# TUM-PIK-ESM/Terrarium.jl

Measured on AMD Instinct MI355X. Metric: column-steps/sec, higher is better.
Workload: dtype f64

## Files before the change

### terrarium.jl_amd/csrc/terrarium_hip.hip

```cpp
#include "trm_host.hpp"

#include <dlfcn.h>

using namespace trm;
using namespace trmh;

namespace {
thread_local std::string g_create_error;
}

namespace trmh {
int fail(trm_ctx* ctx, int code, const std::string& msg) {
    if (ctx) ctx->err = msg;
    else g_create_error = msg;
    return code;
}
}

namespace {

template <class NF> struct HostGrid {
    std::vector<NF> zF, zC, dzc, rdzc, rdzf, dzf, psiz;
    NF dzf_bot, dzf_top;
    void build(int Nz, const double* thickness) {
// ... 443 lines not shown
            for (const auto& a : c->averages) {
                if (a.field != f) continue;
                if (b.count == ACC_BATCH) return fail(c, TRM_EUNSUPPORTED, "more than 32 accumulators of fields that share a field");
                AccumEntry& e = b.e[b.count++];
                e.src = c->d_acc_partial[sl];
                e.sum = a.d_sum;
                e.n = (long long)field_elems(c, f);
                e.pitch = is_3d(f) ? c->Nzp : 1;
                e.nz = is_3d(f) ? c->Nz : 1;
                e.src_double = 1;
            }
        }
        int rc = TRM_OK;
        by_bool(P::richards(c), [&](auto RICH) { rc = ColumnAccumLaunch<NF, RICH()>::run(c, dt, finalize, nsteps, aa); });
        if (!rc) rc = AverageLaunch<NF>::accumulate(c, b);
        if (rc) return rc;
        for (auto& a : c->averages) {
            if (a.field < 0) continue;
            for (int j = 0; j < nsteps; ++j) a.window += dt;
            a.steps += nsteps;
        }
        return TRM_OK;
    }
    template <int PROG> static int fused_prologue(trm_ctx* c, double dt, int nsteps) {
        if (PROG == PROG_MULTI && !c->series.empty()) return U::upload_series_rows(c, dt, nsteps);
        int rc = U::update_inputs(c, c->state, c->time);
        if (!rc && PROG == PROG_HEUN) rc = U::update_inputs(c, c->stage, c->time + dt);
        return rc;
    }
    template <int PROG> static int step_launch(trm_ctx* c, const StepPlan& plan, double dt, int fin, int nsteps) {
        if (plan.route == ROUTE_SURFACE_IN_LAUNCH) return std::is_same<NF, float>::value ? PackedLaunch::step_land(c, dt, fin) : FrontLaunch::run(c, plan, dt, fin, PROG == PROG_HEUN);
        if (plan.route == ROUTE_ACCUM_IN_LAUNCH) return multi_program_accum(c, dt, fin, nsteps);
        if (plan.route == ROUTE_LEVELS) return levels_launch<NF>(c, PROG, P::generic_bcs(c), dt, fin, nsteps);
        if (plan.route == ROUTE_PACKED) return PackedLaunch::step(c, dt, fin);
        if (plan.route == ROUTE_GENERIC) return PROG == PROG_HEUN ? GenericLaunch<NF>::heun(c, dt, fin) : GenericLaunch<NF>::step(c, dt, fin);
        int rc = TRM_OK;
        by_bool(P::richards(c), [&](auto RICH) { rc = ColumnLaunch<NF, RICH(), PROG>::run(c, plan, dt, fin, nsteps); });
        return rc;
    }
    static int fused_epilogue(trm_ctx* c, int rc, double dt, int fin, bool accumulate = true, bool deferred = false, bool psi_step = false) {
        if (!rc) c->closure_consistent = true;
        c->psi_consistent = !rc && psi_step;
        if (!rc) c->closure_deferred = deferred;
        if (!rc && accumulate) rc = accumulate_after(c, dt);
        c->tend_valid = fin != 0;
        c->top_valid = c->params.seb != 0 && !rc && tops_current(c);
        if (rc || !fin) return rc;
        if (P::coupled(c)) return V::surface_veg(c, c->state, true, false, 0.0);
        return c->params.seb ? U::surface(c, c->state, true) : TRM_OK;
    }
    template <int PROG> static int fused_launch(trm_ctx* c, double dt, int fin, int nsteps = 1, bool not_last = false, bool* interior = nullptr) {
        int rc = fused_prologue<PROG>(c, dt, nsteps);
        const StepPlan plan = P::plan_step(c, PROG, not_last, interior && *interior);
        const bool in_launch = plan.route == ROUTE_SURFACE_IN_LAUNCH, accum = plan.route == ROUTE_ACCUM_IN_LAUNCH;
        const bool surface_reads_fields = c->params.seb && !in_launch && !(c->top_valid && c->d_top3);
        if (!rc && c->closure_deferred && (surface_reads_fields || !plan.derives_unread)) rc = flush_closure(c);
        if (PROG != PROG_EULER && plan.check_entry && !rc) rc = fail(c, TRM_EINVAL, "trm_step: an interior launch must be followed by a ForwardEuler launch");
        if (!rc && plan.refusal) rc = fail(c, TRM_EINVAL, plan.refusal);
        if (!rc && PROG != PROG_MULTI && P::coupled(c)) rc = V::surface_veg(c, c->state, true, true, dt, c->opt_write_kf != 0);
        else if (!rc && PROG != PROG_MULTI && c->params.seb && !in_launch) rc = U::surface(c, c->state, true);
        if (!rc) rc = step_launch<PROG>(c, plan, dt, fin, nsteps);
        if (!rc && plan.psi_form == PSI_INTERIOR) c->interior_launches += 1;
        if (!rc && interior) *interior = plan.psi_form == PSI_INTERIOR;
        return fused_epilogue(c, rc, dt, fin, !accum, !plan.store_closure, plan.psi_step);
    }
    static bool interleave_now(trm_ctx* c, int steps_left) {
        if (c->opt_pipeline == 0 || steps_left < 2 || averaging(c) || !c->params.seb || !P::richards(c) || P::coupled(c) || c->part_n[1] <= 0) return false;
        if (!c->series.empty() || P::generic_bcs(c) || c->Nz > 64) return false;
        if (std::is_same<NF, float>::value && !P::packed_path(c)) return false;
        return c->opt_pipeline == 1;
    }
    static int land_steps_interleaved(trm_ctx* c, double dt, int nsteps, int finalize) {
        const bool top0 = c->top_valid, cc0 = c->closure_consistent;
        int rc = flush_closure(c);
        if (rc) return rc;
        {
            PartScope scope(c, 0);
            c->top_valid = top0;
            rc = U::surface(c, c->state, true);
        }
        for (int n = 0; n < nsteps && !rc; ++n) {
            const int fin = (finalize && n == nsteps - 1) ? 1 : 0;
            const bool tops = (n == 0) ? top0 : tops_current(c);
            c->closure_consistent = (n == 0) ? cc0 : true;
            rc = LandLaunch<NF>::run(c, 0, 1, dt, fin, tops);
            if (rc) break;
            if (n < nsteps - 1) {
                rc = LandLaunch<NF>::run(c, 1, 0, dt, 0, tops_current(c));
            } else {
                PartScope scope(c, 1);
                rc = step_launch<PROG_EULER>(c, P::plan_step(c, PROG_EULER, false, false), dt, fin, 1);
            }
            tick(c, dt, 1);
        }
        return fused_epilogue(c, rc, dt, finalize);
    }
    static int steps_per_launch_now(trm_ctx* c) {
        return !program_applies(c) ? 1 : (c->opt_steps_per_launch > 0 ? c->opt_steps_per_launch : P::auto_steps_per_launch(c));
    }
    static int step(trm_ctx* c, double dt, int nsteps, int finalize) {
        if (c->veg_mode == TRM_VEGETATION_STANDALONE) return veg_step(c, dt, nsteps, finalize, false);
        if (c->opt_kernel != TRM_KERNEL_FUSED || P::levels_per_lane(c) == 0)
            if (int rf = flush_closure(c)) return rf;
        const bool fused = c->opt_kernel == TRM_KERNEL_FUSED && P::levels_per_lane(c) > 0;
        const bool program_ok = program_applies(c);
        const bool avg = averaging(c), avg_in_launch = avg && program_ok && averages_in_launch(c);
        const int spl = (avg && !avg_in_launch) ? 1 : steps_per_launch_now(c);
        int n = 0, rc = TRM_OK;
        bool behind_interior = false;
        while (n < nsteps && !rc) {
            int m = std::min(spl, nsteps - n);
            const int fin = (finalize && n + m == nsteps) ? 1 : 0;
            if (!fused) {
                rc = U::update_inputs(c, c->state, c->time);
                c->top_valid = false;
                c->tend_valid = true;
                if (!rc) rc = unfused_step(c, dt, fin);
                if (!rc) c->closure_consistent = true;
                c->psi_consistent = false;
            } else if (m > 1 || (program_ok && single_step_program(c))) {
                rc = fused_launch<PROG_MULTI>(c, dt, fin, m, false, &behind_interior);
            } else if (interleave_now(c, nsteps - n)) {
                m = nsteps - n;
                rc = land_steps_interleaved(c, dt, m, finalize);
                n += m;
                continue;
            } else {
                rc = fused_launch<PROG_EULER>(c, dt, fin, 1, n + m < nsteps && !fin, &behind_interior);
            }
            if (rc) break;
            tick(c, dt, m);
            n += m;
        }
        if (behind_interior) {
            c->psi_consistent = false;
            const std::string err = c->err;
            if (!flush_closure(c) && !U::closure_hydrology(c, c->state, true, false)) (void)U::hydraulics(c, c->state);
            c->err = err;
            if (!rc) rc = fail(c, TRM_EINVAL, "trm_step: the call ended on an interior launch");
        }
        return rc;
    }

    static int copy_state_to_stage(trm_ctx* c, bool everything = false) {
        for (int f = 0; f < TRM_FIELD_COUNT; ++f) {
            if (!c->state.f[f] || !c->stage.f[f]) continue;
            if (f == TRM_FIELD_VWC_FORCING && c->stage_vwc_own) continue;
            const bool needed = everything || !is_3d(f) || f == TRM_FIELD_INTERNAL_ENERGY || f == TRM_FIELD_SATURATION_WATER_ICE ||
                                f == TRM_FIELD_TEND_INTERNAL_ENERGY || f == TRM_FIELD_TEND_SATURATION_WATER_ICE;
            if (needed) TRM_HIP(c, hipMemcpyAsync(c->stage.f[f], c->state.f[f], field_elems(c, f) * sizeof(NF), hipMemcpyDeviceToDevice, c->stream));
        }
        if (everything && c->state.kf_top && c->stage.kf_top)
            TRM_HIP(c, hipMemcpyAsync(c->stage.kf_top, c->state.kf_top, (size_t)c->Nh * sizeof(NF), hipMemcpyDeviceToDevice, c->stream));
        return TRM_OK;
    }
    static int heun_step_coupled_fused(trm_ctx* c, double dt, int finalize) {
        int rc = fused_prologue<PROG_HEUN>(c, dt, 1);
        if (!rc) rc = flush_closure(c);
        if (rc) return fused_epilogue(c, rc, dt, finalize);
        const VegView<NF> vs = P::veg_view(c, c->state);
        VegView<NF> vg = P::veg_view(c, c->stage);
        View<NF> sv = cached_view<NF>(c, c->stage);
        auto fed = [&](int field) {
            for (const auto& sr : c->series) if (!sr.is_bc && sr.field == field) return true;
            return false;
// ... 89 lines not shown
        c->closure_consistent = true;
        c->psi_consistent = false;
        c->last_program = TRM_PROGRAM_UNFUSED;
        int rc = heun_predict(c, dt);
        if (!rc) rc = heun_correct(c, dt, finalize);
        return rc;
    }
};

#define DISPATCH(c, expr) ((c)->precision == TRM_F64 ? Ops<double>::expr : Ops<float>::expr)

bool parse_env_int(const char* name, long lo, long hi, long multiple_of, long& out, std::string& err) {
    const char* e = std::getenv(name);
    if (!e) return false;
    char* end = nullptr;
    const long v = std::strtol(e, &end, 10);
    if (end == e || *end != 0 || v < lo || v > hi || (multiple_of > 1 && v % multiple_of != 0)) {
        err = std::string(name) + "=" + e + ": expected an integer in [" + std::to_string(lo) + ", " + std::to_string(hi) + "]" +
              (multiple_of > 1 ? " that is a multiple of " + std::to_string(multiple_of) : std::string());
        return false;
    }
    out = v;
    return true;
}
struct EnvSwitches {
    long field_skew = 16640, derive_default = -1, debug_placement = 0, handoff_tag_bias = 0, defer_closure = -1, interior_steps = -1;
    std::string error;
    EnvSwitches() {
        long v;
        if (parse_env_int("TRM_FIELD_SKEW", 0, 1 << 20, 256, v, error)) field_skew = v;
        if (error.empty() && parse_env_int("TRM_DERIVE_DEFAULT", 0, 5, 1, v, error)) derive_default = v;
        if (error.empty() && parse_env_int("TRM_DEBUG_PLACEMENT", 0, 1, 1, v, error)) debug_placement = v;
        if (error.empty() && parse_env_int("TRM_DEBUG_HANDOFF_TAG_BIAS", 0, 1, 1, v, error)) handoff_tag_bias = v;
        if (error.empty() && parse_env_int("TRM_DEFER_CLOSURE_STORES", 0, 1, 1, v, error)) defer_closure = v;
        if (error.empty() && parse_env_int("TRM_INTERIOR_STEPS", 0, 2, 1, v, error)) interior_steps = v;
        if (error.empty() && parse_env_int("TRM_STAGED_SMALL", 0, 1, 1, v, error)) {  }
        if (error.empty() && parse_env_int("TRM_SCALAR_INPUTS", 0, 1, 1, v, error)) {  }
    }
};
const EnvSwitches& env_switches() {
    static const EnvSwitches e;
    return e;
}
size_t field_skew_bytes() { return (size_t)env_switches().field_skew; }
int alloc_fields(trm_ctx* c, FieldSet& s) {
    for (int f = 0; f < TRM_FIELD_COUNT; ++f) {
        if (is_lazy_field(f) && c->veg_mode == TRM_VEGETATION_OFF) continue;
        if (s.f[f]) continue;
        size_t bytes = field_elems(c, f) * c->esize;
        const size_t skew = field_skew_bytes() * (size_t)(f % 32);
        TRM_HIP(c, hipMalloc(&s.raw[f], bytes + skew));
        s.f[f] = (char*)s.raw[f] + skew;
        if (env_switches().debug_placement) std::fprintf(stderr, "trm placement: field %d raw %p bytes %zu skew %zu\n", f, s.raw[f], bytes, skew);
        TRM_HIP(c, hipMemsetAsync(s.f[f], 0, bytes, c->stream));
    }
    if (!s.kf_top) {
        TRM_HIP(c, hipMalloc(&s.kf_top, (size_t)c->Nh * c->esize));
        TRM_HIP(c, hipMemsetAsync(s.kf_top, 0, (size_t)c->Nh * c->esize, c->stream));
    }
    TRM_HIP(c, hipStreamSynchronize(c->stream));
    return TRM_OK;
}

template <class NF> int upload_grid(trm_ctx* c, const double* thickness) {
    HostGrid<NF> g;
    g.build(c->Nz, thickness);
    auto up = [&](void** d, const std::vector<NF>& h) -> int {
// ... 1678 lines not shown
        if (int rf = flush_closure(c)) return rf;
    }
    switch (option) {
        case TRM_OPT_ASYNC: c->opt_async = value != 0; return TRM_OK;
        case TRM_OPT_STEP_KERNEL:
            if (value != TRM_KERNEL_FUSED && value != TRM_KERNEL_UNFUSED) break;
            c->opt_kernel = value;
            return TRM_OK;
        case TRM_OPT_WRITE_KF_EVERY_STEP: c->opt_write_kf = value != 0; return TRM_OK;
        case TRM_OPT_VWC_FORCING_FIELD: c->opt_vwc_field = value != 0; return TRM_OK;
        case TRM_OPT_PACKED_F32: c->opt_packed = value != 0; return TRM_OK;
        case TRM_OPT_DERIVE_CLOSURE_FIELDS:
            if (value < 0 || value > 5) break;
            c->opt_derive = value;
            return TRM_OK;
        case TRM_OPT_STEPS_PER_LAUNCH:
            if (value < 0 || value > 100000) break;
            c->opt_steps_per_launch = value;
            return TRM_OK;
        case TRM_OPT_PIPELINE_PARTS:
            if (value < 0 || value > 2) break;
            c->opt_pipeline = value;
            return TRM_OK;
        case TRM_OPT_SINGLE_STEP_PROGRAM:
            if (value < 0 || value > 2) break;
            c->opt_single_step = value;
            return TRM_OK;
        case TRM_OPT_BC_SIGNATURE: c->opt_bc_signature = value != 0; return TRM_OK;
        case TRM_OPT_ZERO_GRADIENT_FAST: c->opt_zero_gradient_fast = value != 0; c->args_valid = false; return TRM_OK;
        case TRM_OPT_SURFACE_IN_LAUNCH:
            if (value < 0 || value > 2) break;
            c->opt_front = value;
            return TRM_OK;
        case TRM_OPT_DEFER_CLOSURE_STORES: c->opt_defer_closure = value != 0; return TRM_OK;
        case TRM_OPT_INTERIOR_STEPS:
            if (value < 0 || value > 2) break;
            c->opt_interior = value;
            return TRM_OK;
        case TRM_OPT_DERIVATIVE_SERIES: c->opt_derivative_series = value != 0; return TRM_OK;
        case TRM_OPT_DERIVATIVE_SERIES_PARAMS: c->opt_derivative_series_params = value != 0; return TRM_OK;
        default: break;
    }
    return fail(c, TRM_EINVAL, "trm_set_option: unknown option or value");
}
int trm_get_option(const trm_ctx* c, int option, int* value) {
    if (!c || !value) return TRM_EINVAL;
    switch (option) {
        case TRM_OPT_ASYNC: *value = c->opt_async; return TRM_OK;
        case TRM_OPT_STEP_KERNEL: *value = c->opt_kernel; return TRM_OK;
        case TRM_OPT_WRITE_KF_EVERY_STEP: *value = c->opt_write_kf; return TRM_OK;
        case TRM_OPT_VWC_FORCING_FIELD: *value = c->opt_vwc_field; return TRM_OK;
        case TRM_OPT_PACKED_F32: *value = c->opt_packed; return TRM_OK;
        case TRM_OPT_DERIVE_CLOSURE_FIELDS: *value = c->opt_derive; return TRM_OK;
        case TRM_OPT_STEPS_PER_LAUNCH: *value = c->opt_steps_per_launch; return TRM_OK;
        case TRM_OPT_PIPELINE_PARTS: *value = c->opt_pipeline; return TRM_OK;
        case TRM_OPT_SINGLE_STEP_PROGRAM: *value = c->opt_single_step; return TRM_OK;
        case TRM_OPT_BC_SIGNATURE: *value = c->opt_bc_signature; return TRM_OK;
        case TRM_OPT_ZERO_GRADIENT_FAST: *value = c->opt_zero_gradient_fast; return TRM_OK;
        case TRM_OPT_SURFACE_IN_LAUNCH: *value = c->opt_front; return TRM_OK;
        case TRM_OPT_DEFER_CLOSURE_STORES: *value = c->opt_defer_closure; return TRM_OK;
        case TRM_INFO_CLOSURE_STORED: *value = c->closure_deferred ? 0 : 1; return TRM_OK;
        case TRM_INFO_MATERIALIZATIONS: *value = (int)c->materializations; return TRM_OK;
        case TRM_OPT_INTERIOR_STEPS: *value = c->opt_interior; return TRM_OK;
        case TRM_INFO_INTERIOR_LAUNCHES: *value = (int)c->interior_launches; return TRM_OK;
        case TRM_OPT_DERIVATIVE_SERIES: *value = c->opt_derivative_series; return TRM_OK;
        case TRM_OPT_DERIVATIVE_SERIES_PARAMS: *value = c->opt_derivative_series_params; return TRM_OK;
        case TRM_INFO_DERIVATIVE_SERIES: *value = c->derivative_series; return TRM_OK;
// ... 23 lines not shown
```

### terrarium.jl_amd/csrc/trm_host.hpp

```cpp
#pragma once
#include "../../include/terrarium_hip.h"
#include "trm_kernels.hpp"
#include "trm_column.hpp"
#include "trm_vegetation.hpp"
#include "trm_dispatch.hpp"

#include <rccl/rccl.h>

#include <cmath>
#include <limits>
#include <type_traits>
#include <cstdio>
#include <cstdlib>
#include <cstring>
#include <algorithm>
#include <string>
#include <vector>

struct FieldSet {
    void* f[TRM_FIELD_COUNT];
    void* kf_top;
    void* raw[TRM_FIELD_COUNT];
};

// ... 655 lines not shown
template <class NF, bool RICH, int H, int LPC, bool SEB, bool SERIES>
int run_column_accum(trm_ctx* c, dim3 grid, dim3 block, const View<NF>& v, const DevParams<NF>& p, const ColumnArgs<NF>& a, const AccumArgs& acc) {
    TRM_LAUNCH(c, (k_column_accum<NF, RICH, H, LPC, SEB, SERIES>), grid, block, v, p, a, acc);
    c->last_program = program_id(TRM_PROGRAM_COLUMN_MULTI, H, LPC, DERIVE_NONE, 0, 1, BCSIG_RUNTIME) | (SEB ? 1 << 25 : 0) | (SERIES ? 1 << 26 : 0) | TRM_PROGRAM_AVERAGES_IN_LAUNCH;
    return TRM_OK;
}
template <int H, int LPC, int DERIVE, bool STAGED, bool SCALAR_IN, int PROG>
int run_column_land(trm_ctx* c, dim3 grid, dim3 block, const View<double>& v, const DevParams<double>& p, const ColumnArgs<double>& a, const FrontArgs& fa) {
    TRM_LAUNCH(c, (k_column_land<double, true, H, LPC, DERIVE, STAGED, SCALAR_IN, PROG>), grid, block, v, p, a, fa);
    c->last_program = program_id(TRM_PROGRAM_COLUMN_LAND, H, LPC, DERIVE, STAGED, SCALAR_IN, BCSIG_LAND) | (PROG << 25);
    return TRM_OK;
}
template <class NF, bool RICH, int SIG> struct ColumnSigLaunch {
    static int run(trm_ctx* c, dim3 grid, dim3 block, const View<NF>& v, const DevParams<NF>& p, const ColumnArgs<NF>& a, int derive, int staged, int scalar_in);
};
template <int SIG> struct ColumnPsiLaunch {
    static int run(trm_ctx* c, dim3 grid, dim3 block, const View<double>& v, const DevParams<double>& p, const ColumnArgs<double>& a, int form, int staged, int scalar_in);
};
template <class NF, bool RICH, int SIG> struct ColumnSigHeunLaunch {
    static int run(trm_ctx* c, dim3 grid, dim3 block, const View<NF>& v, const DevParams<NF>& p, const ColumnArgs<NF>& a);
};
template <class NF> struct GenericLaunch {
    static int step(trm_ctx* c, double dt, int finalize);
    static int heun(trm_ctx* c, double dt, int finalize);
};
template <class NF, int M> struct LevelsLaunch { static int run(trm_ctx* c, int prog, bool generic, double dt, int finalize, int nsteps); };
template <class NF> inline int levels_launch(trm_ctx* c, int prog, bool generic, double dt, int finalize, int nsteps = 1) {
    return Policy<NF>::levels_per_lane(c) == 4 ? LevelsLaunch<NF, 4>::run(c, prog, generic, dt, finalize, nsteps) : LevelsLaunch<NF, 2>::run(c, prog, generic, dt, finalize, nsteps);
}
template <class NF> struct LandLaunch { static int run(trm_ctx* c, int qcol, int qsurf, double dt, int finalize, bool top_arrays); };
template <> int LandLaunch<double>::run(trm_ctx* c, int qcol, int qsurf, double dt, int finalize, bool top_arrays);
template <> int LandLaunch<float>::run(trm_ctx* c, int qcol, int qsurf, double dt, int finalize, bool top_arrays);
struct PackedLaunch {
    static int step(trm_ctx* c, double dt, int finalize);
    static int step_land(trm_ctx* c, double dt, int finalize);
};
int front_args(trm_ctx* c, const char* kernel, FrontArgs& fa);
struct FrontLaunch {
    static int run(trm_ctx* c, const StepPlan& plan, double dt, int finalize, bool heun = false);
    template <int H> static int run_hyd(trm_ctx* c, const StepPlan& plan, double dt, int finalize, bool heun);
};

#ifndef TRM_SINGLE_STEP_PROGRAM_MAX_COLUMNS
#define TRM_SINGLE_STEP_PROGRAM_MAX_COLUMNS 0
#endif

constexpr int kAccumField[ACC_SLOTS] = {
    TRM_FIELD_INTERNAL_ENERGY, TRM_FIELD_SATURATION_WATER_ICE, TRM_FIELD_TEMPERATURE, TRM_FIELD_LIQUID_WATER_FRACTION, TRM_FIELD_PRESSURE_HEAD,
    TRM_FIELD_SURFACE_EXCESS_WATER, TRM_FIELD_WATER_TABLE, TRM_FIELD_SKIN_TEMPERATURE, TRM_FIELD_GROUND_HEAT_FLUX, TRM_FIELD_SURFACE_SHORTWAVE_UP,
    TRM_FIELD_SURFACE_LONGWAVE_UP, TRM_FIELD_SURFACE_NET_RADIATION, TRM_FIELD_SENSIBLE_HEAT_FLUX, TRM_FIELD_LATENT_HEAT_FLUX,
    TRM_FIELD_EVAPORATION_GROUND, TRM_FIELD_INFILTRATION, TRM_FIELD_SURFACE_RUNOFF};
inline int accum_slot(int field) {
    for (int s = 0; s < ACC_SLOTS; ++s) if (kAccumField[s] == field) return s;
    return -1;
}
inline int accum_field(int slot) { return kAccumField[slot]; }

template <class NF> struct StepPolicy : Policy<NF> {
    using P = Policy<NF>;
    static bool tops_current(const trm_ctx* c) { return c->d_top3 != nullptr && !c->top_escaped; }
    static bool averaging(const trm_ctx* c) {
        for (const auto& a : c->averages) if (a.field >= 0) return true;
        return false;
    }
    static bool averages_in_launch(const trm_ctx* c) {
        if (c->Nz > 64 || c->part >= 0) return false;
// ... 13 lines not shown
    static bool interior_capable(const trm_ctx* c) {
        if (!std::is_same<NF, double>::value || !c->opt_interior || !c->psi_consistent || c->closure_escaped) return false;
        if (c->opt_interior == 2 && (size_t)6 * (size_t)c->Nh * (size_t)c->Nzp * sizeof(NF) > ((size_t)256 << 20)) return false;
        if (!c->opt_write_kf) return false;
        if (!P::richards(c) || c->params.seb || P::coupled(c) || c->veg_mode == TRM_VEGETATION_STANDALONE) return false;
        if (c->opt_kernel != TRM_KERNEL_FUSED || P::levels_per_lane(c) != 1 || c->part >= 0 || P::generic_bcs(c)) return false;
        if (!c->opt_bc_signature || P::hyd(c) == HYD_GENERIC || !column_psi_supported(bc_signature_of(c))) return false;
        if (averaging(c) || c->d_tan[0]) return false;
        return P::template derive_now<true>(c) == DERIVE_T_LIQ;
    }
    static bool surface_in_launch(const trm_ctx* c, bool heun = false) {
        if (c->opt_front == 0 || (heun && std::is_same<NF, float>::value)) return false;
        if (!c->params.seb || !P::richards(c) || P::coupled(c) || c->Nz > 64 || P::generic_bcs(c) || c->part >= 0) return false;
        if (c->opt_kernel != TRM_KERNEL_FUSED || !c->opt_bc_signature || bc_signature_of(c) != BCSIG_LAND) return false;
        if (P::hyd(c) != HYD_BC_LINEAR && P::hyd(c) != HYD_VG_N2) return false;
        if (!c->top_valid || !tops_current(c)) return false;
        const int d = heun ? DERIVE_NONE : P::template derive_now<true>(c);
        if (std::is_same<NF, float>::value ? !(P::packed_path(c) && (d == DERIVE_NONE || d == DERIVE_LIQ))
                                           : !(d == DERIVE_NONE || d == DERIVE_T_LIQ)) return false;
        if (c->opt_front == 1) return true;
        return c->Nh <= (std::is_same<NF, float>::value ? 32768 : 65536);
    }
    static bool single_step_program(const trm_ctx* c) {
        if (!c->params.seb || c->Nz > 64 || c->opt_single_step == 0) return false;
        if (c->opt_single_step == 1) return true;
        return c->Nh <= TRM_SINGLE_STEP_PROGRAM_MAX_COLUMNS;
    }
    static int auto_steps_per_launch(const trm_ctx*) { return 50; }
    static bool program_applies(const trm_ctx* c) {
        const bool fused = c->opt_kernel == TRM_KERNEL_FUSED && P::levels_per_lane(c) > 0;
        return fused && !P::generic_bcs(c) && !P::coupled(c) && c->veg_mode != TRM_VEGETATION_STANDALONE &&
               ((c->Nz <= 64 && P::series_fit_program(c)) || (P::levels_per_lane(c) == 2 && !c->params.seb && c->series.empty()));
    }
    static StepPlan plan_step(const trm_ctx* c, int prog, bool not_last, bool behind_interior) {
        StepPlan s;
        const bool rich = P::richards(c), in_launch = prog != PROG_MULTI && surface_in_launch(c, prog == PROG_HEUN);
        if (in_launch) s.route = ROUTE_SURFACE_IN_LAUNCH;
        else if (prog == PROG_MULTI && averaging(c) && averages_in_launch(c)) s.route = ROUTE_ACCUM_IN_LAUNCH;
        else if (P::levels_per_lane(c) > 1) s.route = ROUTE_LEVELS;
        else if (prog == PROG_EULER && P::packed_path(c)) s.route = ROUTE_PACKED;
        else if (prog != PROG_MULTI && P::generic_bcs(c)) s.route = ROUTE_GENERIC;
        if (prog == PROG_EULER && (s.route == ROUTE_COLUMN || (in_launch && std::is_same<NF, double>::value))) {
            s.derive = rich ? P::template derive_now<true>(c) : P::template derive_now<false>(c);
            s.sig = (c->opt_bc_signature && P::hyd(c) != HYD_GENERIC) ? bc_signature_of(c) : -1;
            if (s.derive == DERIVE_T_LIQ) s.staged = rich ? P::template staged_now<true>(c) : P::template staged_now<false>(c);
            if (s.derive == DERIVE_T_LIQ) s.scalar_in = rich ? P::template scalar_inputs_now<true>(c) : P::template scalar_inputs_now<false>(c);
            const bool has_instance = signature_has_instance(s.sig, rich);
            P::io_paths(!has_instance || s.sig == BCSIG_LAND, s.staged, s.scalar_in);
            s.derives_unread = s.derive == DERIVE_T_LIQ && c->part < 0;
            s.store_closure = defer_closure_now(c, s.derives_unread) ? 0 : 1;
            s.psi_step = !in_launch && rich;
        }
        s.check_entry = behind_interior ? 1 : 0;
        if (prog == PROG_EULER && (behind_interior || not_last)) {
            const bool capable = !in_launch && interior_capable(c);
            if (capable && not_last && !s.store_closure) s.psi_form = PSI_INTERIOR;
            else if (behind_interior && capable) s.psi_form = PSI_LAST;
            else if (behind_interior) s.refusal = "trm_step: the launch behind an interior launch cannot derive the pressure head";
        }
        return s;
    }
};

}
```

### terrarium.jl_amd/csrc/trm_launch_packed.hip

```cpp
#include "trm_host.hpp"
#include "trm_packed_f32.hpp"

namespace trmh {

template <int LPC> static unsigned packed_blocks(long n) {
    const long pairs = (n + 1) / 2;
    const long waves = (pairs + (64 / LPC) - 1) / (64 / LPC);
    return (unsigned)((waves * 64 + TRM_STEP_BLOCK - 1) / TRM_STEP_BLOCK);
}
template <bool RICH, int LPC, int H, int DERIVE, int BCSIG = BCSIG_RUNTIME> static int run_packed(trm_ctx* c, double dt, int finalize, int staged) {
    const LaunchArgs<float>& la = launch_args<float>(c);
    TRM_LAUNCH(c, (k_step_pk<RICH, LPC, H, DERIVE, BCSIG>), dim3(packed_blocks<LPC>(ncols(c))), dim3(TRM_STEP_BLOCK), state_view<float>(c), la.p, (float)dt, finalize, write_kf(c, finalize), staged);
    c->last_program = program_id(TRM_PROGRAM_PACKED_F32, H, LPC, DERIVE, staged, 1, BCSIG);
    return TRM_OK;
}
int PackedLaunch::step(trm_ctx* c, double dt, int finalize) {
    using P = Policy<float>;
    int rc = NO_INSTANCE;
    by_bool(P::richards(c), [&](auto RICH) { by_lanes(c->Nz, [&](auto LPC) { by_compiled_hyd(P::hyd(c), [&](auto H) {
        const int derive = P::derive_now<RICH()>(c);
        const int staged = P::staged_now<RICH()>(c, true);
        if constexpr (RICH()) {
            if (derive == DERIVE_LIQ && c->opt_bc_signature)
                by_packed_signature(bc_signature_of(c), [&](auto SIG) { rc = run_packed<true, LPC(), H(), DERIVE_LIQ, SIG()>(c, dt, finalize, staged); });
        }
        if (rc == NO_INSTANCE)
            by_value<DERIVE_NONE, DERIVE_T_LIQ, DERIVE_LIQ, DERIVE_LIQ_PSI>(derive, [&](auto D) { rc = run_packed<RICH(), LPC(), H(), D()>(c, dt, finalize, staged); });
    }); }); });
    return launched(c, rc, "k_step_pk: no instance for this launch");
}

template <int LPC, int H, int DERIVE> static int run_packed_land(trm_ctx* c, const FrontArgs& fa, double dt, int finalize, int staged) {
    const LaunchArgs<float>& la = launch_args<float>(c);
    TRM_LAUNCH(c, (k_step_pk_land<LPC, H, DERIVE>), dim3((unsigned)fa.chain_blocks + packed_blocks<LPC>(c->Nh)), dim3(TRM_STEP_BLOCK), la.state, la.p, (float)dt, finalize, write_kf(c, finalize), staged, fa);
    c->last_program = program_id(TRM_PROGRAM_PACKED_LAND, H, LPC, DERIVE, staged, 1, BCSIG_LAND);
    return TRM_OK;
}
int PackedLaunch::step_land(trm_ctx* c, double dt, int finalize) {
    using P = Policy<float>;
    FrontArgs fa;
    if (int rc = front_args(c, "k_step_pk_land", fa)) return rc;
    const int derive = P::derive_now<true>(c), staged = P::staged_now<true>(c, true);
    if (derive != DERIVE_NONE && derive != DERIVE_LIQ) return fail(c, TRM_EINVAL, "k_step_pk_land: no instance for this derivation mode");
    int rc = NO_INSTANCE;
    by_lanes(c->Nz, [&](auto LPC) { by_compiled_hyd(P::hyd(c), [&](auto H) { by_value<DERIVE_NONE, DERIVE_LIQ>(derive, [&](auto D) {
        rc = run_packed_land<LPC(), H(), D()>(c, fa, dt, finalize, staged);
    }); }); });
    return launched(c, rc, "k_step_pk_land: no instance for the generic hydraulics");
}

template <int H, int LPC, bool TOP_ARRAYS> static int run_land_pk(trm_ctx* c, int qcol, int qsurf, double dt, int finalize) {
    const LaunchArgs<float>& la = launch_args<float>(c);
    const unsigned sblocks = (unsigned)((c->part_n[qsurf] + TRM_STEP_BLOCK - 1) / TRM_STEP_BLOCK);
    TRM_LAUNCH(c, (k_land_pk<true, LPC, H, TOP_ARRAYS>), dim3(sblocks + packed_blocks<LPC>(c->part_n[qcol])), dim3(TRM_STEP_BLOCK), la.part[qcol], la.p, (float)dt, finalize, write_kf(c, finalize), la.part[qsurf], (int)sblocks);
    c->last_program = program_id(TRM_PROGRAM_LAND_INTERLEAVED, H, LPC, DERIVE_NONE, 0, 1, -1);
    return TRM_OK;
}
template <> int LandLaunch<float>::run(trm_ctx* c, int qcol, int qsurf, double dt, int finalize, bool top_arrays) {
    if (top_arrays && !launch_args<float>(c).part[qsurf].top_T) return fail(c, TRM_EINVAL, "LandModel launch: the top-cell arrays were requested on a context that has none");
    int rc = NO_INSTANCE;
    by_compiled_hyd(Policy<float>::hyd(c), [&](auto H) { by_lanes(c->Nz, [&](auto LPC) { by_bool(top_arrays, [&](auto TOPS) {
        rc = run_land_pk<H(), LPC(), TOPS()>(c, qcol, qsurf, dt, finalize);
    }); }); });
// ... 5 lines not shown
```

### terrarium.jl_amd/csrc/trm_packed_f32.hpp

```cpp
#pragma once
#include "trm_kernels.hpp"

namespace trm {
namespace pk {

typedef float v2f __attribute__((ext_vector_type(2)));
struct M2 { bool x, y; };

TRM_DEV v2f splat(float a) { return v2f{a, a}; }
TRM_DEV v2f sel(M2 m, v2f a, v2f b) { return v2f{m.x ? a.x : b.x, m.y ? a.y : b.y}; }
TRM_DEV v2f sel(bool m, v2f a, v2f b) { return v2f{m ? a.x : b.x, m ? a.y : b.y}; }
TRM_DEV M2 lt(v2f a, v2f b) { return M2{a.x < b.x, a.y < b.y}; }
TRM_DEV M2 ge(v2f a, v2f b) { return M2{a.x >= b.x, a.y >= b.y}; }
TRM_DEV M2 eq(v2f a, v2f b) { return M2{a.x == b.x, a.y == b.y}; }
TRM_DEV M2 operator||(M2 a, M2 b) { return M2{a.x || b.x, a.y || b.y}; }
TRM_DEV v2f fma2(v2f a, v2f b, v2f c) { return __builtin_elementwise_fma(a, b, c); }
TRM_DEV v2f min2(v2f a, v2f b) { return v2f{jl_min(a.x, b.x), jl_min(a.y, b.y)}; }
TRM_DEV v2f max2(v2f a, v2f b) { return v2f{jl_max(a.x, b.x), jl_max(a.y, b.y)}; }
TRM_DEV v2f div2(v2f a, v2f b) { return v2f{div_nr(a.x, b.x), div_nr(a.y, b.y)}; }
TRM_DEV v2f up2(v2f a) { return v2f{shift_up(a.x), shift_up(a.y)}; }
TRM_DEV v2f dn2(v2f a) { return v2f{shift_dn(a.x), shift_dn(a.y)}; }
TRM_DEV v2f ld2(const float* base, unsigned off0, unsigned off1) { return v2f{ldg(base, off0), ldg(base, off1)}; }

TRM_DEV v2f div_const2(v2f a, float b, float rb) {
// ... 120 lines not shown
    const v2f r = div_const2_nsz(theta - p.theta_res, p.theta_span, p.rtheta_span);
    const v2f v = pow_int_m5_2(r) * (-p.bc_psi_s);
    const v2f psim = sel(lt(theta, splat(p.por)), v, splat(-p.bc_psi_s));
    const v2f psih = max2(splat(0.0f), z0 - z);
    return psih + psim + psiz;
}
template <int HYD> TRM_DEV v2f conductivity_hydraulic2(const DevParams<float>& p, v2f liq, const Frac2& f) {
    if (HYD == HYD_BC_LINEAR) return conductivity_linear2(p, f);
    return v2f{conductivity_vg<float, false, true>(p, liq.x, Frac<float>{f.water.x, f.ice.x, f.air.x}),
               conductivity_vg<float, false, true>(p, liq.y, Frac<float>{f.water.y, f.ice.y, f.air.y})};
}
template <int HYD> TRM_DEV v2f pressure_head_hyd2(const DevParams<float>& p, v2f sat, float z, float psiz, v2f z0) {
    if (HYD == HYD_BC_LINEAR) return pressure_head2(p, sat, z, psiz, z0);
    return v2f{pressure_head<float, HYD_VG_N2, true>(p, sat.x, z, psiz, z0.x), pressure_head<float, HYD_VG_N2, true>(p, sat.y, z, psiz, z0.y)};
}
TRM_DEV v2f upwind2(v2f g, v2f Kdn, v2f Kmid, v2f Kup) { return min2(Kmid, sel(lt(g, splat(0.0f)), Kdn, Kup)); }

}

struct FrontGranulesF {
    unsigned long long w[3];
    TRM_DEV void load(const unsigned long long* gran, unsigned byte_off_uniform) {
        for (int n = 0; n < 3; ++n) w[n] = sld_off<unsigned long long>(gran, byte_off_uniform + (unsigned)n * 8u);
    }
    TRM_DEV unsigned mismatch(unsigned epoch) const {
        unsigned bad = ((unsigned)(w[0] >> 32) ^ epoch) | ((unsigned)(w[1] >> 32) ^ epoch) | ((unsigned)(w[2] >> 32) ^ epoch);
        asm volatile("" : "+s"(bad));
        return bad;
    }
    TRM_DEV float value(int q) const { return __builtin_bit_cast(float, (unsigned)w[q]); }
};
template <bool RICHARDS, int LPC, int HYD, int DERIVE = DERIVE_NONE, int BCSIG = BCSIG_RUNTIME, bool FRONT = false>
TRM_DEV void step_pk_program(const View<float>& v_arg, const DevParams<float>& p_arg, float dt, int finalize, int write_kf, unsigned block, int staged = 0,
                             const FrontArgs* fa = nullptr) {
    static_assert(!FRONT || (BCSIG == BCSIG_LAND && RICHARDS), "the in-launch surface processes feed the LandModel step");
    constexpr unsigned off_p = round_up_to((unsigned)sizeof(View<float>), (unsigned)alignof(DevParams<float>));
    const View<float>& v = v_arg;
    const DevParams<float>& p = p_arg;
    using namespace pk;
    typedef float NF;
    constexpr int CPW = 64 / LPC;
    TRM_PHASE("addressing");
    const int lane = threadIdx.x & 63;
#if TRM_CUT_MASKS
    const int wave = __builtin_amdgcn_readfirstlane((int)((block * (unsigned)TRM_STEP_BLOCK + threadIdx.x) >> 6));
    const int k = lane % LPC, sub = lane / LPC;
    const int Nz = v.Nz, Nh = (int)v.Nh;
    const bool upper = CPW == 2 && lane_in(0xffffffff00000000ull);
    const unsigned long long m_bot = level_lanes<LPC>(0), m_top = level_lanes<LPC>(Nz - 1);
    const bool is_bot = lane_in(m_bot), is_top = lane_in(m_top);
    const LevelGeom<NF> L = level_geom(v, k);
    const bool need_kc = RICHARDS || write_kf;

    const int pair_w0 = wave * CPW * 2;
    const int i0 = pair_w0 + sub * 2, i1 = i0 + 1;
    const unsigned long long half_lo = CPW == 1 ? ~0ull : 0x00000000ffffffffull, half_hi = CPW == 1 ? 0ull : 0xffffffff00000000ull;
    const unsigned long long m_lev = levels_below<LPC>(Nz);
    const unsigned long long m_act0 = ((pair_w0 < Nh ? half_lo : 0ull) | (pair_w0 + 2 < Nh ? half_hi : 0ull)) & m_lev;
    const unsigned long long m_act1 = ((pair_w0 + 1 < Nh ? half_lo : 0ull) | (pair_w0 + 3 < Nh ? half_hi : 0ull)) & m_lev;
    const bool act0 = lane_in(m_act0), act1 = lane_in(m_act1);
    const int j0 = i0 < Nh ? i0 : Nh - 1, j1 = i1 < Nh ? i1 : Nh - 1;
#else
    const int wave = (int)((block * (unsigned)blockDim.x + threadIdx.x) >> 6);
    const int k = lane % LPC, sub = lane / LPC;
    const int Nz = v.Nz, Nh = (int)v.Nh;
    const bool upper = sub != 0;
    const bool is_bot = k == 0, is_top = k == Nz - 1;
// ... 172 lines not shown
#else
    gU += flux_U;
    if (RICHARDS) gS += flux_S;
#endif
    TRM_PHASE_FENCE("advance", gU, gS, Kf_lo);
    const v2f Unew = U + gU * dt;
    bool bad = (act0 && is_nan(Unew.x)) || (act1 && is_nan(Unew.y));
    v2f snew = sat, z0 = splat(0.0f), GS_top = splat(0.0f), S_out = splat(0.0f);
    if (RICHARDS) {
        snew = sat + gS * dt;
        bad = bad || (act0 && is_nan(snew.x)) || (act1 && is_nan(snew.y));
        float sx = snew.x, sy = snew.y;
        const float over0 = repair_saturation<NF, LPC>(v, sx, k, Nz, m_act0, is_bot, is_top, L, m_bot, m_top);
        const float over1 = repair_saturation<NF, LPC>(v, sy, k, Nz, m_act1, is_bot, is_top, L, m_bot, m_top);
        snew = v2f{sx, sy};
        z0 = v2f{water_table<NF, LPC>(sx, m_act0, lane, L), water_table<NF, LPC>(sy, m_act1, lane, L)};
        GS_top = v2f{0.0f + jl_min(0.0f, S_in.x), 0.0f + jl_min(0.0f, S_in.y)};
        S_out = v2f{(S_in.x + GS_top.x * dt) + over0, (S_in.y + GS_top.y * dt) + over1};
    }
    TRM_PHASE_FENCE("closure", snew, z0, S_out, GS_top);
    v2f ln, Tn;
    const DevParams<float>& p2 = kernarg_reload<DevParams<float>>(off_p);
    const Frac2 f_new = energy_closure2<RICHARDS ? 2 : 1>(p2, Unew, snew, ln, Tn, viol);
    const v2f psin = RICHARDS ? pressure_head_hyd2<HYD>(p2, snew, L.zC, L.psiz, z0) : splat(0.0f);
    TRM_PHASE_FENCE("outputs", ln, Tn);
    v2f Kf_out = Kf_lo, Kf_out_top = Kc;
    if (finalize && write_kf) {
        const v2f Kc_new = conductivity_hydraulic2<HYD>(p, ln, f_new);
        const v2f Kmin_new = min2(Kc_new, up2(Kc_new));
        Kf_out = sel(is_bot || is_top, Kc_new, Kmin_new);
        Kf_out_top = Kc_new;
    }
    constexpr int cpb = (TRM_STEP_BLOCK / 64) * CPW * 2;
    auto store = [&](bool act, int cib, unsigned cb_, unsigned ib_, float u, float t, float l, float s, float ps, float kf, float kft, float gu, float gs,
                     float S_new, float GS, float wt, float Ts_old ) {
        if (!act) return;
        if (is_top && staged) {
            float* st = small_stage<float>();
            if (write_kf) st[SMALL_KF_TOP * cpb + cib] = kft;
            if (RICHARDS) {
                if (finalize) st[SMALL_G_S * cpb + cib] = GS;
                st[SMALL_S * cpb + cib] = S_new;
                st[SMALL_WT * cpb + cib] = wt;
            }
            if (seb) {
                st[SMALL_TS * cpb + cib] = Ts_old;
                st[SMALL_TOP_T * cpb + cib] = t;
                st[SMALL_TOP_SAT * cpb + cib] = s;
                st[SMALL_TOP_LIQ * cpb + cib] = l;
            }
        } else if (is_top) {
            if (RICHARDS) {
                if (finalize) stg(v.G_S, block_local(ib_), GS);
                const unsigned ib = block_local(ib_);
                stg(v.S, ib, S_new);
                stg(v.wt, ib, wt);
            }
            if (seb) stg(v.Ts, block_local(ib_), Ts_old);
        }
        if (finalize) {
            const unsigned cb = block_local(cb_);
            stg(v.G_U, cb, gu);
            if (RICHARDS) stg(v.G_sat, cb, gs);
        }
        {
            const unsigned cb = block_local(cb_);
            stg(v.U, cb, u);
            stg(v.T, cb, t);
            stg(v.liq, cb, l);
            if (RICHARDS) { stg(v.sat, cb, s); stg(v.psi, cb, ps); }
        }
        if (is_top && seb && !staged) { const unsigned ib = block_local(ib_); stg(v.top_T, ib, t); stg(v.top_sat, ib, s); stg(v.top_liq, ib, l); }
        if (write_kf) {
            stg(v.Kf, block_local(cb_), kf);
            if (is_top && !staged) stg(v.Kf_top, block_local(ib_), kft);
        }
    };
    v2f Ts_new = splat(0.0f);
    if (seb) Ts_new = Ts_in + splat(0.0f) * dt;
    asm volatile("" : "+v"(Ts_new), "+v"(S_out), "+v"(GS_top));
    TRM_PHASE("stores");
    const int cib0 = ((int)(threadIdx.x >> 6) * CPW + sub) * 2;
    store(act0, cib0, cb0, ib0, Unew.x, Tn.x, ln.x, snew.x, psin.x, Kf_out.x, Kf_out_top.x, gU.x, gS.x, S_out.x, GS_top.x, z0.x, Ts_new.x);
    store(act1, cib0 + 1, cb1, ib1, Unew.y, Tn.y, ln.y, snew.y, psin.y, Kf_out.y, Kf_out_top.y, gU.y, gS.y, S_out.y, GS_top.y, z0.y, Ts_new.y);
    if (staged) {
        const unsigned enabled = (write_kf ? 1u << SMALL_KF_TOP : 0u) | (RICHARDS ? (1u << SMALL_S) | (1u << SMALL_WT) : 0u) |
                                 ((RICHARDS && finalize) ? 1u << SMALL_G_S : 0u) |
                                 (seb ? (1u << SMALL_TOP_T) | (1u << SMALL_TOP_SAT) | (1u << SMALL_TOP_LIQ) | (1u << SMALL_TS) : 0u);
        store_small_outputs<float, cpb>(enabled, block, Nh);
    }
    const uint32_t flags = (bad ? 1u : 0u) | ((((viol & 2u) && act0) || ((viol & 4u) && act1)) ? 2u : 0u) | (front_timeout ? 4u : 0u);
    if (flags) atomicOr(v.status, flags);
}
template <bool RICHARDS, int LPC, int HYD, int DERIVE = DERIVE_NONE, int BCSIG = BCSIG_RUNTIME>
__global__ void __launch_bounds__(TRM_STEP_BLOCK) k_step_pk(View<float> v_arg, DevParams<float> p_arg, float dt, int finalize, int write_kf, int staged) {
    step_pk_program<RICHARDS, LPC, HYD, DERIVE, BCSIG>(v_arg, p_arg, dt, finalize, write_kf, xcd_block<TRM_XCD_REMAP_PK != 0>(blockIdx.x, gridDim.x), staged);
}
template <int LPC, int HYD, int DERIVE>
__global__ void __launch_bounds__(TRM_STEP_BLOCK) k_step_pk_land(View<float> v_arg, DevParams<float> p_arg, float dt, int finalize, int write_kf, int staged, FrontArgs fa) {
    const int chain_blocks = (int)((v_arg.Nh + (TRM_STEP_BLOCK - 1)) / TRM_STEP_BLOCK);
    if ((int)blockIdx.x < chain_blocks) {
        __builtin_amdgcn_s_setprio(3);
        const long i = (long)blockIdx.x * TRM_STEP_BLOCK + threadIdx.x;
        constexpr unsigned off_p = round_up_to((unsigned)sizeof(View<float>), (unsigned)alignof(DevParams<float>));
        constexpr unsigned off_fa = round_up_to(off_p + (unsigned)sizeof(DevParams<float>) + 4u * (unsigned)sizeof(int), (unsigned)alignof(FrontArgs));
        const View<float>& v = kernarg_reload<View<float>>(0);
        if (i - (long)(threadIdx.x & 63u) < v.Nh) surface_front<float, true, HYD>(v, kernarg_reload<DevParams<float>>(off_p), kernarg_reload<FrontArgs>(off_fa), i);
        return;
    }
    step_pk_program<true, LPC, HYD, DERIVE, BCSIG_LAND, true>(v_arg, p_arg, dt, finalize, write_kf, blockIdx.x - (unsigned)chain_blocks, staged, &fa);
}
template <bool RICHARDS, int LPC, int HYD, bool TOP_ARRAYS>
__global__ void __launch_bounds__(TRM_STEP_BLOCK) k_land_pk(View<float> v_col, DevParams<float> p_arg, float dt, int finalize, int write_kf, View<float> v_surf, int surface_blocks) {
    if ((int)blockIdx.x < surface_blocks) {
        const long i = (long)blockIdx.x * blockDim.x + threadIdx.x;
        if (i < v_surf.Nh) surface_program<float, RICHARDS, HYD, true, TOP_ARRAYS>(v_surf, p_arg, i);
        return;
    }
    step_pk_program<RICHARDS, LPC, HYD, DERIVE_NONE>(v_col, p_arg, dt, finalize, write_kf, blockIdx.x - (unsigned)surface_blocks);
}

}
```

Measured before the change: 3.498 billion.

## Skip T/liq stores in packed f32 inner launches and rederive them next step

Adds a packed-launch plan that, for Richards runs with deferred closure stores, switches inner launches to DERIVE_T_LIQ and skips writing T and liq, since the next launch rederives them from U/sat. This targets global store bandwidth on large states. It is gated by state size over 256 MiB with linear hydraulics, or by a new opt level 2. The plan threads an 'unstored' flag across launches and fails a call that ends on an unstored launch.

```diff
diff --git a/terrarium.jl_amd/csrc/terrarium_hip.hip b/terrarium.jl_amd/csrc/terrarium_hip.hip
--- a/terrarium.jl_amd/csrc/terrarium_hip.hip
+++ b/terrarium.jl_amd/csrc/terrarium_hip.hip
@@ -499,7 +499,7 @@
         if (plan.route == ROUTE_SURFACE_IN_LAUNCH) return std::is_same<NF, float>::value ? PackedLaunch::step_land(c, dt, fin) : FrontLaunch::run(c, plan, dt, fin, PROG == PROG_HEUN);
         if (plan.route == ROUTE_ACCUM_IN_LAUNCH) return multi_program_accum(c, dt, fin, nsteps);
         if (plan.route == ROUTE_LEVELS) return levels_launch<NF>(c, PROG, P::generic_bcs(c), dt, fin, nsteps);
-        if (plan.route == ROUTE_PACKED) return PackedLaunch::step(c, dt, fin);
+        if (plan.route == ROUTE_PACKED) return PackedLaunch::step(c, plan, dt, fin);
         if (plan.route == ROUTE_GENERIC) return PROG == PROG_HEUN ? GenericLaunch<NF>::heun(c, dt, fin) : GenericLaunch<NF>::step(c, dt, fin);
         int rc = TRM_OK;
         by_bool(P::richards(c), [&](auto RICH) { rc = ColumnLaunch<NF, RICH(), PROG>::run(c, plan, dt, fin, nsteps); });
@@ -516,9 +516,9 @@
         if (P::coupled(c)) return V::surface_veg(c, c->state, true, false, 0.0);
         return c->params.seb ? U::surface(c, c->state, true) : TRM_OK;
     }
-    template <int PROG> static int fused_launch(trm_ctx* c, double dt, int fin, int nsteps = 1, bool not_last = false, bool* interior = nullptr) {
+    template <int PROG> static int fused_launch(trm_ctx* c, double dt, int fin, int nsteps = 1, bool not_last = false, bool* interior = nullptr, bool* unstored = nullptr) {
         int rc = fused_prologue<PROG>(c, dt, nsteps);
-        const StepPlan plan = P::plan_step(c, PROG, not_last, interior && *interior);
+        const StepPlan plan = P::plan_step(c, PROG, not_last, interior && *interior, unstored && *unstored);
         const bool in_launch = plan.route == ROUTE_SURFACE_IN_LAUNCH, accum = plan.route == ROUTE_ACCUM_IN_LAUNCH;
         const bool surface_reads_fields = c->params.seb && !in_launch && !(c->top_valid && c->d_top3);
         if (!rc && c->closure_deferred && (surface_reads_fields || !plan.derives_unread)) rc = flush_closure(c);
@@ -529,6 +529,7 @@
         if (!rc) rc = step_launch<PROG>(c, plan, dt, fin, nsteps);
         if (!rc && plan.psi_form == PSI_INTERIOR) c->interior_launches += 1;
         if (!rc && interior) *interior = plan.psi_form == PSI_INTERIOR;
+        if (!rc && unstored) *unstored = plan.route == ROUTE_PACKED && !plan.store_closure;
         return fused_epilogue(c, rc, dt, fin, !accum, !plan.store_closure, plan.psi_step);
     }
     static bool interleave_now(trm_ctx* c, int steps_left) {
@@ -575,6 +576,7 @@
         const int spl = (avg && !avg_in_launch) ? 1 : steps_per_launch_now(c);
         int n = 0, rc = TRM_OK;
         bool behind_interior = false;
+        bool behind_unstored = false;
         while (n < nsteps && !rc) {
             int m = std::min(spl, nsteps - n);
             const int fin = (finalize && n + m == nsteps) ? 1 : 0;
@@ -586,18 +588,24 @@
                 if (!rc) c->closure_consistent = true;
                 c->psi_consistent = false;
             } else if (m > 1 || (program_ok && single_step_program(c))) {
-                rc = fused_launch<PROG_MULTI>(c, dt, fin, m, false, &behind_interior);
+                rc = fused_launch<PROG_MULTI>(c, dt, fin, m, false, &behind_interior, &behind_unstored);
             } else if (interleave_now(c, nsteps - n)) {
                 m = nsteps - n;
                 rc = land_steps_interleaved(c, dt, m, finalize);
                 n += m;
                 continue;
             } else {
-                rc = fused_launch<PROG_EULER>(c, dt, fin, 1, n + m < nsteps && !fin, &behind_interior);
+                rc = fused_launch<PROG_EULER>(c, dt, fin, 1, n + m < nsteps && !fin, &behind_interior, &behind_unstored);
             }
             if (rc) break;
             tick(c, dt, m);
             n += m;
+        }
+        if (behind_unstored) {
+            const std::string err = c->err;
+            (void)flush_closure(c);
+            c->err = err;
+            if (!rc) rc = fail(c, TRM_EINVAL, "trm_step: the call ended on a launch that left T / liq unstored");
         }
         if (behind_interior) {
             c->psi_consistent = false;
@@ -753,7 +761,7 @@
         if (error.empty() && parse_env_int("TRM_DERIVE_DEFAULT", 0, 5, 1, v, error)) derive_default = v;
         if (error.empty() && parse_env_int("TRM_DEBUG_PLACEMENT", 0, 1, 1, v, error)) debug_placement = v;
         if (error.empty() && parse_env_int("TRM_DEBUG_HANDOFF_TAG_BIAS", 0, 1, 1, v, error)) handoff_tag_bias = v;
-        if (error.empty() && parse_env_int("TRM_DEFER_CLOSURE_STORES", 0, 1, 1, v, error)) defer_closure = v;
+        if (error.empty() && parse_env_int("TRM_DEFER_CLOSURE_STORES", 0, 2, 1, v, error)) defer_closure = v;
         if (error.empty() && parse_env_int("TRM_INTERIOR_STEPS", 0, 2, 1, v, error)) interior_steps = v;
         if (error.empty() && parse_env_int("TRM_STAGED_SMALL", 0, 1, 1, v, error)) {  }
         if (error.empty() && parse_env_int("TRM_SCALAR_INPUTS", 0, 1, 1, v, error)) {  }
@@ -2498,7 +2506,7 @@
             if (value < 0 || value > 2) break;
             c->opt_front = value;
             return TRM_OK;
-        case TRM_OPT_DEFER_CLOSURE_STORES: c->opt_defer_closure = value != 0; return TRM_OK;
+        case TRM_OPT_DEFER_CLOSURE_STORES: c->opt_defer_closure = value == 2 ? 2 : value != 0; return TRM_OK;
         case TRM_OPT_INTERIOR_STEPS:
             if (value < 0 || value > 2) break;
             c->opt_interior = value;
diff --git a/terrarium.jl_amd/csrc/trm_host.hpp b/terrarium.jl_amd/csrc/trm_host.hpp
--- a/terrarium.jl_amd/csrc/trm_host.hpp
+++ b/terrarium.jl_amd/csrc/trm_host.hpp
@@ -711,6 +711,7 @@
 template <> int LandLaunch<double>::run(trm_ctx* c, int qcol, int qsurf, double dt, int finalize, bool top_arrays);
 template <> int LandLaunch<float>::run(trm_ctx* c, int qcol, int qsurf, double dt, int finalize, bool top_arrays);
 struct PackedLaunch {
+    static int step(trm_ctx* c, const StepPlan& plan, double dt, int finalize);
     static int step(trm_ctx* c, double dt, int finalize);
     static int step_land(trm_ctx* c, double dt, int finalize);
 };
@@ -790,7 +791,27 @@
         return fused && !P::generic_bcs(c) && !P::coupled(c) && c->veg_mode != TRM_VEGETATION_STANDALONE &&
                ((c->Nz <= 64 && P::series_fit_program(c)) || (P::levels_per_lane(c) == 2 && !c->params.seb && c->series.empty()));
     }
-    static StepPlan plan_step(const trm_ctx* c, int prog, bool not_last, bool behind_interior) {
+    static bool packed_inner_launches(const trm_ctx* c) {
+        if (!std::is_same<NF, float>::value || !P::richards(c) || !defer_closure_now(c, true)) return false;
+        if (P::coupled(c) || c->part >= 0 || !c->closure_consistent || c->closure_escaped) return false;
+        const size_t state_bytes = (size_t)6 * (size_t)c->Nh * (size_t)c->Nzp * sizeof(NF);
+        return c->opt_defer_closure == 2 || (state_bytes > ((size_t)256 << 20) && P::hyd(c) == HYD_BC_LINEAR);
+    }
+    static StepPlan packed_plan(const trm_ctx* c, bool not_last, bool behind_unstored) {
+        StepPlan s;
+        const bool rich = P::richards(c);
+        s.route = ROUTE_PACKED;
+        s.derive = rich ? P::template derive_now<true>(c) : P::template derive_now<false>(c);
+        s.staged = rich ? P::template staged_now<true>(c, true) : P::template staged_now<false>(c, true);
+        s.sig = (rich && s.derive == DERIVE_LIQ && c->opt_bc_signature) ? bc_signature_of(c) : -1;
+        if (s.derive == DERIVE_LIQ && (not_last || behind_unstored) && packed_inner_launches(c)) {
+            s.derive = DERIVE_T_LIQ;
+            s.derives_unread = true;
+            s.store_closure = not_last ? 0 : 1;
+        }
+        return s;
+    }
+    static StepPlan plan_step(const trm_ctx* c, int prog, bool not_last, bool behind_interior, bool behind_unstored = false) {
         StepPlan s;
         const bool rich = P::richards(c), in_launch = prog != PROG_MULTI && surface_in_launch(c, prog == PROG_HEUN);
         if (in_launch) s.route = ROUTE_SURFACE_IN_LAUNCH;
@@ -798,6 +819,7 @@
         else if (P::levels_per_lane(c) > 1) s.route = ROUTE_LEVELS;
         else if (prog == PROG_EULER && P::packed_path(c)) s.route = ROUTE_PACKED;
         else if (prog != PROG_MULTI && P::generic_bcs(c)) s.route = ROUTE_GENERIC;
+        if (s.route == ROUTE_PACKED) s = packed_plan(c, not_last, behind_unstored);
         if (prog == PROG_EULER && (s.route == ROUTE_COLUMN || (in_launch && std::is_same<NF, double>::value))) {
             s.derive = rich ? P::template derive_now<true>(c) : P::template derive_now<false>(c);
             s.sig = (c->opt_bc_signature && P::hyd(c) != HYD_GENERIC) ? bc_signature_of(c) : -1;
diff --git a/terrarium.jl_amd/csrc/trm_launch_packed.hip b/terrarium.jl_amd/csrc/trm_launch_packed.hip
--- a/terrarium.jl_amd/csrc/trm_launch_packed.hip
+++ b/terrarium.jl_amd/csrc/trm_launch_packed.hip
@@ -8,27 +8,30 @@
     const long waves = (pairs + (64 / LPC) - 1) / (64 / LPC);
     return (unsigned)((waves * 64 + TRM_STEP_BLOCK - 1) / TRM_STEP_BLOCK);
 }
-template <bool RICH, int LPC, int H, int DERIVE, int BCSIG = BCSIG_RUNTIME> static int run_packed(trm_ctx* c, double dt, int finalize, int staged) {
+template <bool RICH, int LPC, int H, int DERIVE, int BCSIG = BCSIG_RUNTIME> static int run_packed(trm_ctx* c, double dt, int finalize, int staged, int store_closure) {
     const LaunchArgs<float>& la = launch_args<float>(c);
-    TRM_LAUNCH(c, (k_step_pk<RICH, LPC, H, DERIVE, BCSIG>), dim3(packed_blocks<LPC>(ncols(c))), dim3(TRM_STEP_BLOCK), state_view<float>(c), la.p, (float)dt, finalize, write_kf(c, finalize), staged);
+    TRM_LAUNCH(c, (k_step_pk<RICH, LPC, H, DERIVE, BCSIG>), dim3(packed_blocks<LPC>(ncols(c))), dim3(TRM_STEP_BLOCK), state_view<float>(c), la.p, (float)dt, finalize, write_kf(c, finalize), staged, store_closure);
     c->last_program = program_id(TRM_PROGRAM_PACKED_F32, H, LPC, DERIVE, staged, 1, BCSIG);
     return TRM_OK;
 }
-int PackedLaunch::step(trm_ctx* c, double dt, int finalize) {
+int PackedLaunch::step(trm_ctx* c, const StepPlan& plan, double dt, int finalize) {
     using P = Policy<float>;
+    if (!plan.store_closure && plan.derive != DERIVE_T_LIQ) return fail(c, TRM_EINVAL, "k_step_pk: a launch that reads T / liq must store them");
     int rc = NO_INSTANCE;
     by_bool(P::richards(c), [&](auto RICH) { by_lanes(c->Nz, [&](auto LPC) { by_compiled_hyd(P::hyd(c), [&](auto H) {
-        const int derive = P::derive_now<RICH()>(c);
-        const int staged = P::staged_now<RICH()>(c, true);
+        const int derive = plan.derive, staged = plan.staged, store = plan.store_closure;
         if constexpr (RICH()) {
-            if (derive == DERIVE_LIQ && c->opt_bc_signature)
-                by_packed_signature(bc_signature_of(c), [&](auto SIG) { rc = run_packed<true, LPC(), H(), DERIVE_LIQ, SIG()>(c, dt, finalize, staged); });
+            if (plan.sig >= 0)
+                by_packed_signature(plan.sig, [&](auto SIG) { by_value<DERIVE_LIQ, DERIVE_T_LIQ>(derive, [&](auto D) {
+                    rc = run_packed<true, LPC(), H(), D(), SIG()>(c, dt, finalize, staged, store);
+                }); });
         }
         if (rc == NO_INSTANCE)
-            by_value<DERIVE_NONE, DERIVE_T_LIQ, DERIVE_LIQ, DERIVE_LIQ_PSI>(derive, [&](auto D) { rc = run_packed<RICH(), LPC(), H(), D()>(c, dt, finalize, staged); });
+            by_value<DERIVE_NONE, DERIVE_T_LIQ, DERIVE_LIQ, DERIVE_LIQ_PSI>(derive, [&](auto D) { rc = run_packed<RICH(), LPC(), H(), D()>(c, dt, finalize, staged, store); });
     }); }); });
     return launched(c, rc, "k_step_pk: no instance for this launch");
 }
+int PackedLaunch::step(trm_ctx* c, double dt, int finalize) { return step(c, StepPolicy<float>::packed_plan(c, false, false), dt, finalize); }
 
 template <int LPC, int H, int DERIVE> static int run_packed_land(trm_ctx* c, const FrontArgs& fa, double dt, int finalize, int staged) {
     const LaunchArgs<float>& la = launch_args<float>(c);
diff --git a/terrarium.jl_amd/csrc/trm_packed_f32.hpp b/terrarium.jl_amd/csrc/trm_packed_f32.hpp
--- a/terrarium.jl_amd/csrc/trm_packed_f32.hpp
+++ b/terrarium.jl_amd/csrc/trm_packed_f32.hpp
@@ -176,7 +176,7 @@
 };
 template <bool RICHARDS, int LPC, int HYD, int DERIVE = DERIVE_NONE, int BCSIG = BCSIG_RUNTIME, bool FRONT = false>
 TRM_DEV void step_pk_program(const View<float>& v_arg, const DevParams<float>& p_arg, float dt, int finalize, int write_kf, unsigned block, int staged = 0,
-                             const FrontArgs* fa = nullptr) {
+                             int store_closure = 1, const FrontArgs* fa = nullptr) {
     static_assert(!FRONT || (BCSIG == BCSIG_LAND && RICHARDS), "the in-launch surface processes feed the LandModel step");
     constexpr unsigned off_p = round_up_to((unsigned)sizeof(View<float>), (unsigned)alignof(DevParams<float>));
     const View<float>& v = v_arg;
@@ -415,6 +415,7 @@
         Kf_out_top = Kc_new;
     }
     constexpr int cpb = (TRM_STEP_BLOCK / 64) * CPW * 2;
+    constexpr bool SKIPS_CLOSURE = DERIVE == DERIVE_T_LIQ && !FRONT;
     auto store = [&](bool act, int cib, unsigned cb_, unsigned ib_, float u, float t, float l, float s, float ps, float kf, float kft, float gu, float gs,
                      float S_new, float GS, float wt, float Ts_old ) {
         if (!act) return;
@@ -446,7 +447,10 @@
             stg(v.G_U, cb, gu);
             if (RICHARDS) stg(v.G_sat, cb, gs);
         }
-        {
+        if constexpr (SKIPS_CLOSURE) {
+            { const unsigned cb = block_local(cb_); stg(v.U, cb, u); if (RICHARDS) { stg(v.sat, cb, s); stg(v.psi, cb, ps); } }
+            if (uniform_flag(store_closure)) { const unsigned cb = block_local(cb_); stg(v.T, cb, t); stg(v.liq, cb, l); }
+        } else {
             const unsigned cb = block_local(cb_);
             stg(v.U, cb, u);
             stg(v.T, cb, t);
@@ -476,8 +480,8 @@
     if (flags) atomicOr(v.status, flags);
 }
 template <bool RICHARDS, int LPC, int HYD, int DERIVE = DERIVE_NONE, int BCSIG = BCSIG_RUNTIME>
-__global__ void __launch_bounds__(TRM_STEP_BLOCK) k_step_pk(View<float> v_arg, DevParams<float> p_arg, float dt, int finalize, int write_kf, int staged) {
-    step_pk_program<RICHARDS, LPC, HYD, DERIVE, BCSIG>(v_arg, p_arg, dt, finalize, write_kf, xcd_block<TRM_XCD_REMAP_PK != 0>(blockIdx.x, gridDim.x), staged);
+__global__ void __launch_bounds__(TRM_STEP_BLOCK) k_step_pk(View<float> v_arg, DevParams<float> p_arg, float dt, int finalize, int write_kf, int staged, int store_closure) {
+    step_pk_program<RICHARDS, LPC, HYD, DERIVE, BCSIG>(v_arg, p_arg, dt, finalize, write_kf, xcd_block<TRM_XCD_REMAP_PK != 0>(blockIdx.x, gridDim.x), staged, store_closure);
 }
 template <int LPC, int HYD, int DERIVE>
 __global__ void __launch_bounds__(TRM_STEP_BLOCK) k_step_pk_land(View<float> v_arg, DevParams<float> p_arg, float dt, int finalize, int write_kf, int staged, FrontArgs fa) {
@@ -491,7 +495,7 @@
         if (i - (long)(threadIdx.x & 63u) < v.Nh) surface_front<float, true, HYD>(v, kernarg_reload<DevParams<float>>(off_p), kernarg_reload<FrontArgs>(off_fa), i);
         return;
     }
-    step_pk_program<true, LPC, HYD, DERIVE, BCSIG_LAND, true>(v_arg, p_arg, dt, finalize, write_kf, blockIdx.x - (unsigned)chain_blocks, staged, &fa);
+    step_pk_program<true, LPC, HYD, DERIVE, BCSIG_LAND, true>(v_arg, p_arg, dt, finalize, write_kf, blockIdx.x - (unsigned)chain_blocks, staged, 1, &fa);
 }
 template <bool RICHARDS, int LPC, int HYD, bool TOP_ARRAYS>
 __global__ void __launch_bounds__(TRM_STEP_BLOCK) k_land_pk(View<float> v_col, DevParams<float> p_arg, float dt, int finalize, int write_kf, View<float> v_surf, int surface_blocks) {
```

After: 3.463 billion. 1.0% lower.
